# camillabelponer/dealii-slod

Hardware: AMD Instinct MI355X
Metric: SLOD patches/sec (basis built), 2D Poisson H=1/32 n_sub=8 oversampling 2 (higher is better)
Workload: dtype f64; 1 GPU; C2: 2D Poisson SLOD, H=1/32, n_sub=8, oversampling=2, D1e4 coefficient (contrast 10000), 1024 patches on rank 0 (ensemble of 1 realisations, contiguous patch blocks); patches_per_gpu=1024, parallelism=patch-sharded x1

## Files before the change

dealii-slod_amd/csrc/slod_device.h:

```cpp
#ifndef SLOD_DEVICE_H
#define SLOD_DEVICE_H

#include <hip/hip_runtime.h>
#include <stddef.h>
#include <stdint.h>

struct SlodPatchDesc
{
  int32_t  ox, oy;
  int32_t  nx, ny;
  int32_t  mx, my;
  int32_t  ccx, ccy;
  int32_t  flags;
  int32_t  m, L;
  int32_t  n_c, n_b;
  int32_t  prob;
  uint32_t plan_index;
  uint64_t out_off;
};

__host__ __device__ inline size_t slod_mt_stride(int nc_max) { return (size_t)nc_max * nc_max + 1; }

enum : int32_t
{
  SLOD_F_LOD        = 1 << 4,
  SLOD_F_TRANSPOSED = 1 << 5
};

#ifdef SLOD_ENABLE_DIAG
#define SLOD_DG(A, mask) ((A).diag & (mask))
#else
#define SLOD_DG(A, mask) 0
#endif

struct SlodPatchDiag
{
  int32_t path;
  int32_t n_cut;
  int32_t n_dropped;
  int32_t sweeps;
  double  dinf;
  double  sigma_max, sigma_min;
};

struct SlodKernelArgs
{
  const SlodPatchDesc *desc;
  const double        *coef0;
  const double        *coef1;
  size_t               coef_stride;
  int32_t              NE;
  int32_t              n_sub;
  int32_t              quirk;
  int32_t              diag;
  int32_t              debug;
  double               scale;
  double               invH2;
  double *st;
  size_t  st_stride;
  int32_t nn_max;
  double *vinv;
  size_t  v_stride;
  int32_t m_max;
  int32_t L_max;
  int32_t nv;
  double *xs;
  double *zs;
  size_t  x_stride;
  int32_t nc_max;
  double *ms;
  double *mt;
  int32_t m_tw;
  int32_t bwd_ksplit;
  int32_t nb_buf;
  int32_t nf_max;
  int32_t fuse_select;
  int32_t fuse_assemble;
  double  *basis;
  double  *premult;
  int32_t *status;
  SlodPatchDiag *pdiag;
};

enum SlodSolverKind : int32_t
{
  SLOD_K_MF   = 1,
  SLOD_K_TW   = 2,
  SLOD_K_COOP = 4,
  SLOD_K_ND   = 5
};

struct SlodTuning
{
  int solver = 0;
  int fuse_select = 1, fuse_assemble = 1, fuse_m = -1;
  int twisted = -1;
  int balance = 1;
  int bwd_ksplit = 1;
  int debug = 0;
};
struct SlodSolveChoice
{
  int    kind = 0;
  size_t lds  = 0;
  int    fuse_select = 0, fuse_assemble = 0, m_tw = 0, bwd_ksplit = 0, twisted = 0, debug = 0;
  int    v_line_pad = 0;
  size_t v_line_elems = 0;
  int    nv = 0;
  size_t v_patch_elems = 0;
};
SlodTuning slod_read_tuning();
bool       slod_choose_solver(int S, int n_sub, int m_max, int L_max, int nc_max, int nb_buf, int nf_max, size_t n_patches,
                              const SlodTuning &t, SlodSolveChoice *out);

hipError_t slod_launch_assemble(int S, const SlodKernelArgs &a, int n_patches, hipStream_t st);
hipError_t slod_launch_solve(int S, const SlodSolveChoice &c, SlodKernelArgs &a, int n_patches, hipStream_t st);
hipError_t slod_launch_solve_mf(int S, const SlodKernelArgs &a, int n_patches, size_t lds, hipStream_t st);
hipError_t slod_launch_solve_tw(int S, const SlodKernelArgs &a, int n_patches, size_t lds, hipStream_t st);
hipError_t slod_launch_solve_coop(int S, int twisted, const SlodKernelArgs &a, int n_patches, hipStream_t st);
hipError_t slod_launch_solve_nd(const SlodKernelArgs &a, int n_patches, size_t lds, hipStream_t st);
int        slod_solve_nd_cell(int S, int n_sub, int m_max, int L_max);
size_t     slod_solve_nd_scratch(int nv, int m_max, int L_max, int nc_max);
size_t     slod_solve_nd_lds_bytes(int nv, int m_max, int nc_max);
hipError_t slod_launch_select(int S, const SlodKernelArgs &a, int n_patches, int nb_max,
                              int nf_max, hipStream_t st);
size_t     slod_solve_lds_bytes(int S, int m_max, int nc_max, int twisted);
size_t     slod_solve_tw_lds_bytes(int S, int m_max, int nc_max, bool with_m = false);
size_t     slod_solve_mf_lds_bytes(int S, int m_max, int nc_max);
int        slod_lane_tile(int m_max);
int        slod_solve_mf_tiles(int S, int m_max);
size_t     slod_select_lds_bytes(int S, int nb_max, int nc_max, int nf_max);

#endif
```

dealii-slod_amd/csrc/slod_dispatch.cpp:

```cpp
#include "slod_device.h"

#include <algorithm>
#include <cstdlib>
#include <cstring>

SlodTuning slod_read_tuning()
{
  SlodTuning t;
  if (const char *sel = getenv("SLOD_SOLVE"))
    t.solver = !strcmp(sel, "mf") ? SLOD_K_MF : !strcmp(sel, "tw") ? SLOD_K_TW :
               !strcmp(sel, "coop") ? SLOD_K_COOP : !strcmp(sel, "nd") ? SLOD_K_ND : 0;
  if (const char *e = getenv("SLOD_FUSE_SELECT"))
    t.fuse_select = atoi(e) ? 1 : 0;
  if (const char *e = getenv("SLOD_FUSE_ASSEMBLE"))
    t.fuse_assemble = atoi(e) ? 1 : 0;
  if (const char *e = getenv("SLOD_FUSE_M"))
    t.fuse_m = atoi(e) ? 1 : 0;
  if (const char *e = getenv("SLOD_BWD_KSPLIT"))
    t.bwd_ksplit = atoi(e) ? 1 : 0;
  if (const char *e = getenv("SLOD_TWISTED"))
    t.twisted = atoi(e) ? 1 : 0;
  if (const char *e = getenv("SLOD_BALANCE"))
    t.balance = atoi(e) ? 1 : 0;
  if (const char *e = getenv("SLOD_DEBUG"))
    t.debug = atoi(e) ? 1 : 0;
  return t;
}

int slod_lane_tile(int m_max)
{
  static const int tiles[] = {2, 3, 4, 5, 6, 8, 10, 12, 14};
  for (int t : tiles)
    if (8 * t >= m_max)
      return t;
  return 0;
}

bool slod_choose_solver(int S, int n_sub, int m_max, int L_max, int nc_max, int nb_buf, int nf_max, size_t n_patches,
                        const SlodTuning &t_in, SlodSolveChoice *out)
{
  const size_t    lds_max = 160 * 1024;
  SlodSolveChoice c;
  const int       nd_nv = slod_solve_nd_cell(S, n_sub, m_max, L_max);
  SlodTuning      t     = t_in;
  if (t.solver == SLOD_K_ND && nd_nv == 0)
    t.solver = 0;
  c.debug = t.debug;
  const int  wt = slod_lane_tile(m_max);
  const bool lane_tile_fits = wt > 0 && wt >= 2 * S - 1;
  const auto want = [&](int k) { return t.solver == 0 || t.solver == k; };
  const size_t lds_sel = slod_select_lds_bytes(S, nb_buf, nc_max, nf_max);
  const bool   mf_fits = slod_solve_mf_tiles(S, m_max) > 0 && slod_solve_mf_lds_bytes(S, m_max, nc_max) <= lds_max;
  const bool   tw_fits = lane_tile_fits && slod_solve_tw_lds_bytes(S, m_max, nc_max) <= lds_max;
  if (nd_nv > 0 && t.solver == SLOD_K_ND)
    {
      c.kind          = SLOD_K_ND;
      c.nv            = nd_nv;
      c.lds           = slod_solve_nd_lds_bytes(nd_nv, m_max, nc_max);
      c.v_patch_elems = slod_solve_nd_scratch(nd_nv, m_max, L_max, nc_max);
      c.fuse_assemble = t.fuse_assemble ? 1 : 0;
      c.fuse_select   = 0;
    }
  else if (mf_fits && (t.solver == SLOD_K_MF || (t.solver == 0 && !tw_fits && !lane_tile_fits)))
    {
      c.kind          = SLOD_K_MF;
      c.lds           = slod_solve_mf_lds_bytes(S, m_max, nc_max);
      c.v_line_pad    = 16 * slod_solve_mf_tiles(S, m_max);
      c.v_line_elems  = (size_t)c.v_line_pad * c.v_line_pad;
      c.fuse_assemble = (S == 1 && t.fuse_assemble) ? 1 : 0;
      c.fuse_select   = (S == 1 && t.fuse_select && lds_sel <= lds_max) ? 1 : 0;
      if (c.fuse_select && lds_sel > c.lds)
        c.lds = lds_sel;
    }
  else if (want(SLOD_K_TW) && tw_fits)
    {
      c.kind          = SLOD_K_TW;
      c.lds           = slod_solve_tw_lds_bytes(S, m_max, nc_max);
      c.v_line_pad    = 8 * wt;
      c.v_line_elems  = (size_t)64 * wt * wt;
      c.fuse_assemble = (S == 1 && t.fuse_assemble) ? 1 : 0;
      c.fuse_select = (S == 1 && t.fuse_select && lds_sel <= 64 * 1024) ? 1 : 0;
      if (S == 1 && t.fuse_m != 0 && nc_max <= 32 && 8 * wt <= 48)
        {
          const size_t sel    = c.fuse_select ? lds_sel : 0;
          const size_t with_m = std::max(slod_solve_tw_lds_bytes(S, m_max, nc_max, true), sel);
          if (std::min<size_t>(4, lds_max / with_m) == std::min<size_t>(4, lds_max / std::max(c.lds, sel)))
            {
              c.m_tw = 1;
              c.lds  = slod_solve_tw_lds_bytes(S, m_max, nc_max, true);
            }
        }
      if (c.fuse_select && lds_sel > c.lds)
        c.lds = lds_sel;
      c.bwd_ksplit = (t.bwd_ksplit && 8 * wt <= 48 && nc_max <= 32) ? 1 : 0;
    }
  else if (t.solver == 0 || t.solver == SLOD_K_COOP || !lane_tile_fits)
    {
      int tw = t.twisted >= 0 ? t.twisted : (n_patches < 3 * 256 ? 1 : 0);
      if (slod_solve_lds_bytes(S, m_max, nc_max, tw) > lds_max)
        tw = 0;
      if (slod_solve_lds_bytes(S, m_max, nc_max, tw) > lds_max || (m_max + 15) / 16 > 7)
        return false;
      c.kind       = SLOD_K_COOP;
      c.twisted    = tw;
      c.lds        = slod_solve_lds_bytes(S, m_max, nc_max, tw);
      c.v_line_pad = m_max;
      c.v_line_elems = (size_t)m_max * m_max;
    }
  else
    return false;
  if (!c.fuse_select && lds_sel > lds_max)
    return false;
  *out = c;
  return true;
}

hipError_t slod_launch_solve(int S, const SlodSolveChoice &c, SlodKernelArgs &a, int n_patches, hipStream_t st)
{
  a.m_tw          = c.m_tw;
  a.bwd_ksplit    = c.bwd_ksplit;
  a.fuse_select   = c.fuse_select;
  a.fuse_assemble = c.fuse_assemble;
  a.debug         = c.debug;
  switch (c.kind)
    {
      case SLOD_K_MF:
        return slod_launch_solve_mf(S, a, n_patches, c.lds, st);
      case SLOD_K_TW:
        return slod_launch_solve_tw(S, a, n_patches, c.lds, st);
      case SLOD_K_COOP:
        return slod_launch_solve_coop(S, c.twisted, a, n_patches, st);
      case SLOD_K_ND:
        a.nv = c.nv;
        return slod_launch_solve_nd(a, n_patches, c.lds, st);
      default:
        return hipErrorInvalidValue;
    }
}
```

dealii-slod_amd/csrc/slod_select.hip.h:

```cpp
#ifndef SLOD_SELECT_HIP_H
#define SLOD_SELECT_HIP_H
#include <type_traits>
#include "slod_common.hip.h"

namespace
{

  template <int S, bool OWN = false>
  __device__ __forceinline__ void select_patch(const SlodKernelArgs &A, const int nb_max, const int nf_max,
                                               const int patch, double *smem, const double *mpre = nullptr)
  {
    const SlodPatchDesc d   = A.desc[patch];
    const int           tid = threadIdx.x;
    const int           nc = d.n_c, nb = d.n_b, n = A.n_sub;
    const int           ncm = A.nc_max, ldm = ncm + 1;
    const int           mm = A.m_max, ncs = A.nc_max;
    const bool          tr  = (d.flags & SLOD_F_TRANSPOSED) != 0;
    const bool          lod = (d.flags & SLOD_F_LOD) != 0;
    const int           npx = d.nx + 1, nn = npx * (d.ny + 1), nf = S * nn;

    double *Ms   = smem;
    double *Vj   = Ms + ncm * ldm;
    double *BD   = Vj + ncm * ncm;
    double *phis = BD;
    double *sig  = BD + max(nb_max * ncm, nf_max);
    double *utg  = sig + ncm;
    double *gam  = utg + ncm;
    double *cvec = gam + ncm;
    double *rowk = cvec + ncm;
    double *red  = rowk + ncm;
    const int vst = max(nb_max, 160);
    double *vcol = red + 8;
    int    *colk = reinterpret_cast<int *>(vcol + 2 * vst);
    int    *ord  = colk + 2 * ncm;
    int    *flag = ord + ncm;
    int    *pcol = flag + 4;

    const double *st    = A.st + (size_t)patch * A.st_stride;
    const double *xg    = A.xs + (size_t)patch * A.x_stride;
    const size_t  xline = (size_t)mm * ncs;
    const int     wave = tid >> 6, lane = tid & 63, grp = tid >> 4, l16 = tid & 15;

    auto xrow = [&](int ix, int iy, int comp) -> const double * {
      if (ix <= 0 || ix >= d.nx || iy <= 0 || iy >= d.ny)
        return nullptr;
      const int l = tr ? ix - 1 : iy - 1, pos = tr ? iy - 1 : ix - 1;
      return xg + (size_t)l * xline + (size_t)(pos * S + comp) * ncs;
    };
    auto ptw = [&](int ix, int iy, int comp, int col) -> double {
      if (S == 1)
        {
          const int jx = ix - colk[col] * n, jy = iy - colk[ncm + col] * n;
          if (jx < 0 || jx > n || jy < 0 || jy > n)
            return 0.0;
          return ((jx == 0 || jx == n) ? 1.0 : 2.0) * ((jy == 0 || jy == n) ? 1.0 : 2.0);
        }
      return pt_weight<S>(d, n, A.quirk, ix, iy, comp, col);
    };
    auto block_sum = [&](double v) -> double {
      for (int off = 32; off > 0; off >>= 1)
        v += __shfl_xor(v, off, 64);
      __syncthreads();
      if (lane == 0)
        red[wave] = v;
      __syncthreads();
      return red[0] + red[1] + red[2] + red[3];
    };

    for (int c = tid; c < nc; c += 256)
      {
        int kx, ky;
        cell_of_col(d, c / S, kx, ky);
        colk[c]       = kx;
        colk[ncm + c] = ky;
      }
    __syncthreads();

    const bool stamping = (SLOD_DG(A, (1 << 20))) && tid == 0 && A.nc_max * A.nc_max >= 12;
    double    *msd      = A.ms + (size_t)patch * A.nc_max * A.nc_max;
    double     tph[3]   = {0.0, 0.0, 0.0};
    double     tlast    = stamping ? (double)wall_clock64() : 0.0;
    auto       stamp    = [&](int i) {
      if (stamping)
        msd[i] = tlast = (double)wall_clock64();
    };
    auto tacc = [&](int i) {
      if (stamping)
        {
          const double now = (double)wall_clock64();
          tph[i] += now - tlast;
          tlast = now;
        }
    };

    const bool m_given = mpre != nullptr;
    if (m_given)
      for (int idx = tid; idx < nc * nc; idx += 256)
        Ms[(idx / nc) * ldm + (idx % nc)] = mpre[idx];
    for (int idx = tid; idx < ((SLOD_DG(A, 64)) || m_given ? 0 : nc * (nc + 1) / 2); idx += 256)
      {
        int a = (int)((2.0f * nc + 1.0f - sqrtf((2.0f * nc + 1.0f) * (2.0f * nc + 1.0f) - 8.0f * idx)) * 0.5f);
        a     = min(max(a, 0), nc - 1);
        while (a > 0 && a * (2 * nc - a + 1) / 2 > idx)
          --a;
        while (a + 1 < nc && (a + 1) * (2 * nc - a) / 2 <= idx)
          ++a;
        const int b  = a + idx - a * (2 * nc - a + 1) / 2;
        const int kx = colk[a], ky = colk[ncm + a];
        double    acc = 0.0;
        if (S == 1 || !A.quirk)
          {
            const int ca = a % S;
            for (int jy0 = 0; jy0 <= n; jy0 += 3)
              for (int jx0 = 0; jx0 <= n; jx0 += 9)
                {
                  double xv[3][9];
#pragma unroll
                  for (int ry = 0; ry < 3; ++ry)
                    {
                      const int iy  = ky * n + jy0 + ry;
                      const int iyc = min(max(iy, 1), d.ny - 1);
#pragma unroll
                      for (int rx = 0; rx < 9; ++rx)
                        {
                          const int ix  = kx * n + jx0 + rx;
                          const int ixc = min(max(ix, 1), d.nx - 1);
                          const int l = tr ? ixc - 1 : iyc - 1, pos = tr ? iyc - 1 : ixc - 1;
                          xv[ry][rx]  = xg[(size_t)l * xline + (size_t)(pos * S + ca) * ncs + b];
                        }
                    }
#pragma unroll
                  for (int ry = 0; ry < 3; ++ry)
                    {
                      const int    jy = jy0 + ry, iy = ky * n + jy;
                      const double wy = (jy <= n && iy > 0 && iy < d.ny) ? ((jy == 0 || jy == n) ? 1.0 : 2.0) : 0.0;
                      double       part = 0.0;
#pragma unroll
                      for (int rx = 0; rx < 9; ++rx)
                        {
                          const int    jx = jx0 + rx, ix = kx * n + jx;
                          const double w = (jx <= n && ix > 0 && ix < d.nx) ? ((jx == 0 || jx == n) ? 1.0 : 2.0) : 0.0;
                          part           = fma(w, xv[ry][rx], part);
                        }
                      acc = fma(wy, part, acc);
                    }
                }
          }
        else
          {
            for (int jy = 0; jy <= n; ++jy)
              for (int jx = 0; jx <= n; ++jx)
                {
                  const int ix = kx * n + jx, iy = ky * n + jy;
#pragma unroll
                  for (int c = 0; c < S; ++c)
                    {
                      const double *xr = xrow(ix, iy, c);
                      if (xr)
                        acc = fma(pt_weight<S>(d, n, A.quirk, ix, iy, c, a), xr[b], acc);
                    }
                }
          }
        Ms[a * ldm + b] = acc * A.scale * A.invH2;
        Ms[b * ldm + a] = acc * A.scale * A.invH2;
      }
    __syncthreads();
    stamp(3);

    if (nc * nc <= 1024)
      {
        double mv[4];
        int    mi[4], mj[4];
#pragma unroll
        for (int e = 0; e < 4; ++e)
          {
            const int idx = tid + 256 * e;
            mi[e]         = idx / nc;
            mj[e]         = idx - mi[e] * nc;
            mv[e]         = (idx < nc * nc) ? Ms[mi[e] * ldm + mj[e]] : 0.0;
            if (idx < nc * nc && mi[e] == 0)
              cvec[mj[e]] = mv[e];
          }
        __syncthreads();
        for (int k = 0; k < ((SLOD_DG(A, 128)) ? 0 : nc); ++k)
          {
            const double *rk  = (k & 1) ? rowk : cvec;
            double       *rn  = (k & 1) ? cvec : rowk;
            const double  piv = rk[k];
            if (tid == 0 && !(piv > 0.0) && !SLOD_DG(A, -1))
              atomicOr(A.status, 2);
            const double p = fast_rcp(piv);
#pragma unroll
            for (int e = 0; e < 4; ++e)
              if (tid + 256 * e < nc * nc)
                {
                  const int    i = mi[e], j = mj[e];
                  const double ri = rk[i], rj = rk[j];
                  double       v;
                  if (i == k)
                    v = (j == k) ? -p : rj * p;
                  else if (j == k)
                    v = ri * p;
                  else
                    v = fma(-(ri * rj), p, mv[e]);
                  mv[e] = v;
                  if (i == k + 1)
                    rn[j] = v;
                }
            __syncthreads();
          }
#pragma unroll
        for (int e = 0; e < 4; ++e)
          if (tid + 256 * e < nc * nc)
            Ms[mi[e] * ldm + mj[e]] = -mv[e];
        __syncthreads();
      }
    else
      {
        for (int k = 0; k < ((SLOD_DG(A, 128)) ? 0 : nc); ++k)
          {
            for (int j = tid; j < nc; j += 256)
              rowk[j] = Ms[k * ldm + j];
            __syncthreads();
            const double piv = rowk[k];
            if (tid == 0 && !(piv > 0.0) && !SLOD_DG(A, -1))
              atomicOr(A.status, 2);
            const double p = fast_rcp(piv);
            for (int idx = tid; idx < nc * nc; idx += 256)
              {
                const int    i = idx / nc, j = idx - i * nc;
                const double ri = rowk[i], rj = rowk[j];
                double       v;
                if (i == k)
                  v = (j == k) ? -p : rj * p;
                else if (j == k)
                  v = ri * p;
                else
                  v = fma(-(ri * rj), p, Ms[i * ldm + j]);
                Ms[i * ldm + j] = v;
              }
            __syncthreads();
          }
        for (int idx = tid; idx < nc * nc; idx += 256)
          {
            const int i = idx / nc, j = idx - i * nc;
            Ms[i * ldm + j] = -Ms[i * ldm + j];
          }
        __syncthreads();
      }
    stamp(4);
    double *Ds = Ms;

    for (int dsel = 0; dsel < S; ++dsel)
      {
        for (int j = tid; j < nc; j += 256)
          gam[j] = (j == dsel) ? 1.0 : 0.0;
        SlodPatchDiag pdg = {0, 0, 0, 0, 0.0, 0.0, 0.0};
        if (!lod)
          {
            pdg.path = 1;
            const int nn1 = nc - 1;
            auto      cix = [&](int j) { return j < dsel ? j : j + 1; };
            const int nbuf = nb_max;
            int       nr   = 0;
            bool      need_svd = true, singular = false, did_qr = false;
            int       filled = 0;
            auto qr_sweep = [&](auto &a, const int rows, const bool last) __attribute__((always_inline)) {
              constexpr int RQ = sizeof(a[0]) / sizeof(double);
            if (grp == 0)
              {
                double nx0 = 0.0;
#pragma unroll
                for (int i = 0; i < RQ; ++i)
                  {
                    nx0 = fma(a[0][i], a[0][i], nx0);
                    if (l16 + 16 * i < rows)
                      vcol[l16 + 16 * i] = a[0][i];
                  }
                nx0 = group16_sum(nx0);
                if (l16 == 0)
                  sig[0] = nx0;
              }
            __syncthreads();
            for (int k = 0; k < nn1; ++k)
              {
                const double *vc    = vcol + (k & 1) * vst;
                double       *vn    = vcol + ((k + 1) & 1) * vst;
                const double  sigma = sig[k & 1];
                const bool    act   = sigma > 0.0;
                if (!act && last)
                  singular = true;
                const double x0    = vc[k];
                const double sq    = act ? sigma * fast_rsqrt(sigma) : 0.0;
                const double alpha = (x0 >= 0.0) ? -sq : sq;
                const double v0    = x0 - alpha;
                const double beta  = act ? fast_rcp(sigma - alpha * x0) : 0.0;
                double       vr[RQ];
#pragma unroll
                for (int i = 0; i < RQ; ++i)
                  {
                    const int r = l16 + 16 * i;
                    vr[i]       = (r == k) ? v0 : ((r > k && r < rows) ? vc[r] : 0.0);
                  }
#pragma unroll
                for (int sl = 0; sl < 2; ++sl)
                  {
                    const int j = grp + 16 * sl;
                    if (j == k)
                      {
#pragma unroll
                        for (int i = 0; i < RQ; ++i)
                          {
                            const int r = l16 + 16 * i;
                            a[sl][i]    = (r == k) ? (act ? alpha : a[sl][i]) : (r > k ? 0.0 : a[sl][i]);
                          }
                      }
                    else if (j > k && j <= nn1)
                      {
                        double sd = 0.0;
#pragma unroll
                        for (int i = 0; i < RQ; ++i)
                          sd = fma(vr[i], a[sl][i], sd);
                        sd = group16_sum(sd) * beta;
#pragma unroll
                        for (int i = 0; i < RQ; ++i)
                          a[sl][i] = fma(-sd, vr[i], a[sl][i]);
                        if (j == k + 1 && j < nn1)
                          {
                            double nxt = 0.0;
#pragma unroll
                            for (int i = 0; i < RQ; ++i)
                              {
                                const int r = l16 + 16 * i;
                                if (r > k)
                                  nxt = fma(a[sl][i], a[sl][i], nxt);
                                if (r < rows)
                                  vn[r] = a[sl][i];
                              }
                            nxt = group16_sum(nxt);
                            if (l16 == 0)
                              sig[(k + 1) & 1] = nxt;
                          }
                      }
                  }
                __syncthreads();
              }
            };
            const bool onepass = nb <= 160 && nb > 96 && nc <= 32 && (nbuf & 15) == 0 && !(SLOD_DG(A, (512 | 262144)));
            double     aq[2][10];
            for (int r0 = 0; r0 < nb;)
              {
                const int take = min(nb - r0, nbuf - filled);
                {
                  constexpr int U = 2;
                  for (int idx0 = tid; idx0 < ((SLOD_DG(A, 256)) ? 0 : take * nc); idx0 += 256 * U)
                    {
                      double sv[U][3][S], xv[U][3][S], acc[U];
                      int    dst[U];
#pragma unroll
                      for (int u = 0; u < U; ++u)
                        {
                          const int  idx = idx0 + 256 * u;
                          const bool ok  = idx < take * nc;
                          const int  br = ok ? idx / nc : 0, c = ok ? idx - br * nc : 0;
                          const int  bi = r0 + br;
                          const int  bn = bi / S, ca = bi - bn * S;
                          int        ix, iy;
                          boundary_node(d, bn, ix, iy);
                          acc[u] = -A.scale * ptw(ix, iy, ca, c);
                          dst[u] = ok ? (filled + br) * ncm + c : -1;
                          const bool hor = (iy == 0 || iy == d.ny);
                          const int  ndx = ix == 0 ? 1 : -1, ndy = iy == 0 ? 1 : -1;
#pragma unroll
                          for (int e = -1; e <= 1; ++e)
                            {
                              const int  dx = hor ? e : ndx, dy = hor ? ndy : e;
                              const int  jx = ix + dx, jy = iy + dy;
                              const bool in = (jx > 0 && jx < d.nx && jy > 0 && jy < d.ny);
                              const int  jxc = min(max(jx, 1), d.nx - 1), jyc = min(max(jy, 1), d.ny - 1);
                              const int  dir = (dy + 1) * 3 + dx + 1;
                              const int  l = tr ? jxc - 1 : jyc - 1, pos = tr ? jyc - 1 : jxc - 1;
#pragma unroll
                              for (int cb = 0; cb < S; ++cb)
                                {
                                  const double svv = st[(size_t)((dir * S + ca) * S + cb) * A.nn_max + ix + iy * npx];
                                  sv[u][e + 1][cb] = in ? svv : 0.0;
                                  xv[u][e + 1][cb] = xg[(size_t)l * xline + (size_t)(pos * S + cb) * ncs + c];
                                }
                            }
                        }
#pragma unroll
                      for (int u = 0; u < U; ++u)
                        {
#pragma unroll
                          for (int e = 0; e < 3; ++e)
#pragma unroll
                            for (int cb = 0; cb < S; ++cb)
                              acc[u] = fma(sv[u][e][cb], xv[u][e][cb], acc[u]);
                          if (dst[u] >= 0)
                            BD[dst[u]] = acc[u];
                        }
                    }
                }
                __syncthreads();
                tacc(0);
                for (int ti = wave; 16 * ti < take; ti += 4)
                  {
                    const int  arow = filled + 16 * ti + (lane & 15);
                    const bool aok  = 16 * ti + (lane & 15) < take;
                    double4_t  acc[4];
#pragma unroll
                    for (int tj = 0; tj < 4; ++tj)
                      acc[tj] = double4_t{0.0, 0.0, 0.0, 0.0};
                    for (int k = 0; k < nc; k += 4)
                      {
                        const int    kk = k + (lane >> 4);
                        const double av = (aok && kk < nc) ? BD[arow * ncm + kk] : 0.0;
#pragma unroll
                        for (int tj = 0; tj < 4; ++tj)
                          if (16 * tj < nc)
                            {
                              const int    col = 16 * tj + (lane & 15);
                              const double bv  = (kk < nc && col < nc) ? Ds[kk * ldm + col] : 0.0;
                              acc[tj]          = __builtin_amdgcn_mfma_f64_16x16x4f64(av, bv, acc[tj], 0, 0, 0);
                            }
                      }
#pragma unroll
                    for (int tj = 0; tj < 4; ++tj)
#pragma unroll
                      for (int r = 0; r < 4; ++r)
                        {
                          const int rr = 16 * ti + (lane >> 4) + 4 * r, col = 16 * tj + (lane & 15);
                          if (rr < take && col < nc)
                            BD[(filled + rr) * ncm + col] = acc[tj][r];
                        }
                  }
                __syncthreads();
                tacc(1);
                if (onepass)
                  {
#pragma unroll
                    for (int sl = 0; sl < 2; ++sl)
                      {
                        const int j = grp + 16 * sl, cj = j < nn1 ? cix(j) : dsel;
#pragma unroll
                        for (int i = 0; i < 10; ++i)
                          {
                            const int r = l16 + 16 * i;
                            if (r >= r0 && r < r0 + take)
                              aq[sl][i] = (j <= nn1) ? BD[(r - r0) * ncm + cj] : 0.0;
                            else if (r0 == 0)
                              aq[sl][i] = 0.0;
                          }
                      }
                    r0 += take;
                    __syncthreads();
                    continue;
                  }
                r0 += take;
                const int rows = filled + take;
                nr             = rows;
                if (rows < nn1 || (SLOD_DG(A, 512)))
                  {
                    filled = rows;
                    if (filled >= nbuf)
                      break;
                    continue;
                  }
                did_qr = true;
                if (rows <= 96 && nc <= 32)
                  {
                    double a[2][6];
#pragma unroll
                    for (int sl = 0; sl < 2; ++sl)
                      {
                        const int j = grp + 16 * sl;
                        const int cj = j < nn1 ? cix(j) : dsel;
#pragma unroll
                        for (int i = 0; i < 6; ++i)
                          {
                            const int r = l16 + 16 * i;
                            a[sl][i]    = (j <= nn1 && r < rows) ? BD[r * ncm + cj] : 0.0;
                          }
                      }
                    qr_sweep(a, rows, r0 >= nb);
#pragma unroll
                    for (int sl = 0; sl < 2; ++sl)
                      {
                        const int j = grp + 16 * sl;
                        const int cj = j < nn1 ? cix(j) : dsel;
#pragma unroll
                        for (int i = 0; i < 6; ++i)
                          {
                            const int r = l16 + 16 * i;
                            if (j <= nn1 && r < rows)
                              BD[r * ncm + cj] = a[sl][i];
                          }
                      }
                  }
                else
                  {
                    {
                      double part = 0.0;
                      for (int r = tid; r < rows; r += 256)
                        {
                          const double x = BD[r * ncm + cix(0)];
                          part           = fma(x, x, part);
                        }
                      const double s00 = block_sum(part);
                      if (tid == 0)
                        sig[0] = s00;
                      __syncthreads();
                    }
                    for (int k = 0; k < nn1; ++k)
                      {
                        const int    ck    = cix(k);
                        const double sigma = sig[k & 1];
                        if (!(sigma > 0.0))
                          {
                            if (r0 >= nb)
                              singular = true;
                            if (k + 1 < nn1)
                              {
                                double part = 0.0;
                                for (int r = k + 1 + tid; r < rows; r += 256)
                                  {
                                    const double x = BD[r * ncm + cix(k + 1)];
                                    part           = fma(x, x, part);
                                  }
                                const double sn = block_sum(part);
                                if (tid == 0)
                                  sig[(k + 1) & 1] = sn;
                              }
                            __syncthreads();
                            continue;
                          }
                        const double x0    = BD[k * ncm + ck];
                        const double sq    = sigma * fast_rsqrt(sigma);
                        const double alpha = (x0 >= 0.0) ? -sq : sq;
                        const double v0    = x0 - alpha;
                        const double beta  = fast_rcp(sigma - alpha * x0);
                        if constexpr (OWN)
                          {
                            constexpr int NRL = 10;
                            double        vr[NRL];
    #pragma unroll
                            for (int i = 0; i < NRL; ++i)
                              {
                                const int    r = k + l16 + 16 * i;
                                const double x = BD[min(r, rows - 1) * ncm + ck];
                                vr[i]          = (r < rows) ? ((r == k) ? v0 : x) : 0.0;
                              }
                            for (int t = grp; t < nn1 - k; t += 16)
                              {
                                const int cj = (t == nn1 - k - 1) ? dsel : cix(k + 1 + t);
                                double    xj[NRL];
    #pragma unroll
                                for (int i = 0; i < NRL; ++i)
                                  xj[i] = BD[min(k + l16 + 16 * i, rows - 1) * ncm + cj];
                                double sd = 0.0;
    #pragma unroll
                                for (int i = 0; i < NRL; ++i)
                                  sd = (k + l16 + 16 * i < rows) ? fma(vr[i], xj[i], sd) : sd;
                                sd = group16_sum(sd) * beta;
                                double nxt = 0.0;
    #pragma unroll
                                for (int i = 0; i < NRL; ++i)
                                  {
                                    const int r = k + l16 + 16 * i;
                                    if (r < rows)
                                      {
                                        const double nv  = fma(-sd, vr[i], xj[i]);
                                        BD[r * ncm + cj] = nv;
                                        if (r > k)
                                          nxt = fma(nv, nv, nxt);
                                      }
                                  }
                                if (t == 0 && k + 1 < nn1)
                                  {
                                    nxt = group16_sum(nxt);
                                    if (l16 == 0)
                                      sig[(k + 1) & 1] = nxt;
                                  }
                              }
                          }
                        else
                          {
                            for (int t = grp; t < nn1 - k; t += 16)
                              {
                                const int cj = (t == nn1 - k - 1) ? dsel : cix(k + 1 + t);
                                double    sd = 0.0;
                                for (int r = k + l16; r < rows; r += 16)
                                  {
                                    const double vr = (r == k) ? v0 : BD[r * ncm + ck];
                                    sd              = fma(vr, BD[r * ncm + cj], sd);
                                  }
                                sd = group16_sum(sd) * beta;
                                double nxt = 0.0;
                                for (int r = k + l16; r < rows; r += 16)
                                  {
                                    const double vr = (r == k) ? v0 : BD[r * ncm + ck];
                                    const double nv = fma(-sd, vr, BD[r * ncm + cj]);
                                    BD[r * ncm + cj] = nv;
                                    if (r > k)
                                      nxt = fma(nv, nv, nxt);
                                  }
                                if (t == 0 && k + 1 < nn1)
                                  {
                                    nxt = group16_sum(nxt);
                                    if (l16 == 0)
                                      sig[(k + 1) & 1] = nxt;
                                  }
                              }
                          }
                        __syncthreads();
                        if (tid == 0)
                          BD[k * ncm + ck] = alpha;
                      }
                    for (int idx = tid; idx < nn1 * nn1; idx += 256)
                      {
                        const int r = idx / nn1, j = idx - r * nn1;
                        if (r > j)
                          BD[r * ncm + cix(j)] = 0.0;
                      }
                    for (int r = nn1 + tid; r < rows; r += 256)
                      for (int j = 0; j < nn1; ++j)
                        BD[r * ncm + cix(j)] = 0.0;
                  }
                __syncthreads();
                tacc(2);
                filled = nn1;
                nr     = nn1;
              }
            if (onepass)
              {
                did_qr = true;
                qr_sweep(aq, nb, true);
#pragma unroll
                for (int sl = 0; sl < 2; ++sl)
                  {
                    const int j = grp + 16 * sl, cj = j < nn1 ? cix(j) : dsel;
#pragma unroll
                    for (int i = 0; i < 2; ++i)
                      {
                        const int r = l16 + 16 * i;
                        if (j <= nn1 && r < nn1)
                          BD[r * ncm + cj] = aq[sl][i];
                      }
                  }
                __syncthreads();
                tacc(2);
                nr = nn1;
              }
            if (did_qr && !(SLOD_DG(A, 512)))
              {
                if (!singular)
                  {
                    double    fr = 0.0, fi = 0.0;
                    const int l8 = tid & 7;
                    for (int j = tid >> 3; j < nn1; j += 32)
                      {
                        const int cj = cix(j);
                        if (l8 == 0)
                          Vj[j * nn1 + j] = 1.0 / BD[j * ncm + cj];
                        for (int i = j - 1; i >= 0; --i)
                          {
                            const double rd = fast_rcp(BD[i * ncm + cix(i)]);
                            double       sa = 0.0;
                            for (int k2 = i + 1 + l8; k2 <= j; k2 += 8)
                              sa = fma(BD[i * ncm + cix(k2)], Vj[k2 * nn1 + j], sa);
                            sa += dpp_rot<0xB1>(sa);
                            sa += dpp_rot<0x4E>(sa);
                            sa += dpp_rot<0x141>(sa);
                            if (l8 == 0)
                              Vj[i * nn1 + j] = -sa * rd;
                          }
                        for (int i = l8; i <= j; i += 8)
                          {
                            const double r = BD[i * ncm + cj], x = Vj[i * nn1 + j];
                            fr             = fma(r, r, fr);
                            fi             = fma(x, x, fi);
                          }
                      }
                    const double nr2 = block_sum(fr), ni2 = block_sum(fi);
                    double       del = 0.0;
                    if (tid < nn1)
                      {
                        for (int j = tid; j < nn1; ++j)
                          del = fma(-Vj[tid * nn1 + j], BD[j * ncm + dsel], del);
                        rowk[tid] = del;
                      }
                    double dmax = fabs(del);
                    for (int off = 32; off > 0; off >>= 1)
                      dmax = fmax(dmax, __shfl_xor(dmax, off, 64));
                    __syncthreads();
                    if (lane == 0)
                      red[4 + wave] = dmax;
                    __syncthreads();
                    const double dinf = fmax(fmax(red[4], red[5]), fmax(red[6], red[7]));
                    pdg.dinf          = dinf;
                    if (nr2 * ni2 < 1e14 && dinf < 0.5 - 1e-9)
                      {
                        need_svd = false;
                        if (tid < nn1)
                          gam[cix(tid)] = rowk[tid];
                      }
                  }
              }
            if (stamping)
              {
                msd[5] = tph[0];
                msd[6] = tph[1];
                msd[7] = tph[2];
              }
            stamp(8);
            if (need_svd && !(SLOD_DG(A, (512 | 4096))))
              {
                pdg.path = 2;
                const bool tposed = did_qr && nbuf >= 2 * nn1 + 1;
                double    *Wm     = BD;
                int        wr     = nr;
                int        pb     = 0;
                for (int j = tid; j < nn1; j += 256)
                  pcol[j] = j;
                if (tposed && nc <= 32 && !(SLOD_DG(A, 65536)))
                  {
                    double a[2][2];
                    bool   fin[2] = {false, false};
#pragma unroll
                    for (int sl = 0; sl < 2; ++sl)
                      {
                        const int j = grp + 16 * sl, cj = j < nn1 ? cix(j) : dsel;
#pragma unroll
                        for (int i = 0; i < 2; ++i)
                          {
                            const int r = l16 + 16 * i;
                            a[sl][i]    = (j <= nn1 && r < nn1) ? BD[r * ncm + cj] : 0.0;
                          }
                        const double nrm = group16_sum(fma(a[sl][0], a[sl][0], a[sl][1] * a[sl][1]));
                        if (j < nn1 && l16 == 0)
                          sig[j] = nrm;
                      }
                    __syncthreads();
                    for (int k = 0; k < nn1; ++k)
                      {
                        const int    *pc  = pcol + pb * ncm;
                        int          *pn  = pcol + (1 - pb) * ncm;
                        const double *cnc = (k & 1) ? utg : sig;
                        double       *cnn = (k & 1) ? sig : utg;
                        int    p;
                        double best;
                        {
                          const bool pin = lane >= k && lane < nn1;
                          double     v   = cnc[pc[pin ? lane : k]];
                          int        q   = pin ? lane : 64;
                          v              = pin ? v : -1.0;
                          auto step = [&](auto CTRL_) __attribute__((always_inline)) {
                            constexpr int CTRL = decltype(CTRL_)::value;
                            const double  ov   = dpp_rot<CTRL>(v);
                            const int     oq   = __builtin_amdgcn_mov_dpp(q, CTRL, 0xf, 0xf, false);
                            const bool    take = (ov > v) | ((ov == v) & (oq < q));
                            v                  = take ? ov : v;
                            q                  = take ? oq : q;
                          };
                          step(std::integral_constant<int, 0x128>{});
                          step(std::integral_constant<int, 0x124>{});
                          step(std::integral_constant<int, 0x122>{});
                          step(std::integral_constant<int, 0x121>{});
                          const int    q0 = __builtin_amdgcn_readlane(q, 0), q1 = __builtin_amdgcn_readlane(q, 16);
                          const double v0 = __hiloint2double(__builtin_amdgcn_readlane(__double2hiint(v), 0),
                                                             __builtin_amdgcn_readlane(__double2loint(v), 0));
                          const double v1 = __hiloint2double(__builtin_amdgcn_readlane(__double2hiint(v), 16),
                                                             __builtin_amdgcn_readlane(__double2loint(v), 16));
                          const bool   hi = v1 > v0;
                          best            = hi ? v1 : v0;
                          p               = hi ? q1 : q0;
                        }
                        if (!(best > 0.0))
                          break;
                        const int cp = pc[p];
                        if (tid < nn1)
                          pn[tid] = (tid == k) ? cp : (tid == p ? pc[k] : pc[tid]);
                        const int    ccp   = cix(cp);
                        const double x0    = BD[k * ncm + ccp];
                        const double sq    = best * fast_rsqrt(best);
                        const double alpha = (x0 >= 0.0) ? -sq : sq;
                        const double v0    = x0 - alpha;
                        const double beta  = fast_rcp(best - alpha * x0);
                        double       vr[2];
#pragma unroll
                        for (int i = 0; i < 2; ++i)
                          {
                            const int r = l16 + 16 * i;
                            vr[i]       = (r == k) ? v0 : ((r > k && r < nn1) ? BD[r * ncm + ccp] : 0.0);
                          }
#pragma unroll
                        for (int sl = 0; sl < 2; ++sl)
                          {
                            const int j = grp + 16 * sl, cj = j < nn1 ? cix(j) : dsel;
                            if (j > nn1 || fin[sl])
                              continue;
                            if (j == cp)
                              {
#pragma unroll
                                for (int i = 0; i < 2; ++i)
                                  {
                                    const int r = l16 + 16 * i;
                                    a[sl][i]    = (r == k) ? alpha : (r > k ? 0.0 : a[sl][i]);
                                  }
                                fin[sl] = true;
                              }
                            else
                              {
                                const double sd = group16_sum(fma(vr[0], a[sl][0], vr[1] * a[sl][1])) * beta;
                                double       nrm = 0.0;
#pragma unroll
                                for (int i = 0; i < 2; ++i)
                                  {
                                    const int r = l16 + 16 * i;
                                    a[sl][i]    = fma(-sd, vr[i], a[sl][i]);
                                    if (r > k)
                                      nrm = fma(a[sl][i], a[sl][i], nrm);
                                    if (r >= k && r < nn1)
                                      BD[r * ncm + cj] = a[sl][i];
                                  }
                                nrm = group16_sum(nrm);
                                if (j < nn1 && l16 == 0)
                                  cnn[j] = nrm;
                              }
                          }
                        __syncthreads();
                        pb ^= 1;
                      }
#pragma unroll
                    for (int sl = 0; sl < 2; ++sl)
                      {
                        const int j = grp + 16 * sl, cj = j < nn1 ? cix(j) : dsel;
#pragma unroll
                        for (int i = 0; i < 2; ++i)
                          {
                            const int r = l16 + 16 * i;
                            if (j <= nn1 && r < nn1)
                              BD[r * ncm + cj] = a[sl][i];
                          }
                      }
                  }
                __syncthreads();
                if (stamping && A.nc_max * A.nc_max >= 16)
                  msd[14] = (double)wall_clock64();
                const int *pc = pcol + pb * ncm;
                if (tposed)
                  {
                    Wm = BD + (size_t)nn1 * ncm;
                    for (int idx = tid; idx < nn1 * nn1; idx += 256)
                      {
                        const int i = idx / nn1, j = idx - i * nn1;
                        Wm[i * ncm + j] = (j <= i) ? BD[j * ncm + cix(pc[i])] : 0.0;
                      }
                    for (int j = tid; j < nn1; j += 256)
                      Wm[nn1 * ncm + j] = BD[j * ncm + dsel];
                    wr = nn1;
                  }
                const int wru = tposed ? wr + 1 : wr;
                auto wcol = [&](int j) { return tposed ? j : cix(j); };
                const int nev = (nn1 + 1) & ~1;
                for (int idx = tid; idx < nn1 * nn1; idx += 256)
                  Vj[idx] = ((idx / nn1) == (idx % nn1)) ? 1.0 : 0.0;
                double fro = 0.0;
                for (int idx = tid; idx < wr * nn1; idx += 256)
                  {
                    const double w = Wm[(idx / nn1) * ncm + wcol(idx % nn1)];
                    fro            = fma(w, w, fro);
                  }
                const double tiny = 1e-22 * block_sum(fro);
                if (nev / 2 <= 16 && (SLOD_DG(A, 131072)))
                  {
                    if (wave == 0)
                      {
                        const int l4 = lane & 3, pr = lane >> 2;
                        for (int sweep = 0; sweep < ((SLOD_DG(A, 8192)) ? 3 : 40); ++sweep)
                          {
                            bool any = false;
                            for (int round = 0; round < nev - 1; ++round)
                              {
                                int pa, pb2;
                                if (pr == 0)
                                  {
                                    pa  = nev - 1;
                                    pb2 = round;
                                  }
                                else
                                  {
                                    pa  = round + pr;
                                    pa  = pa >= nev - 1 ? pa - (nev - 1) : pa;
                                    pb2 = round - pr;
                                    pb2 = pb2 < 0 ? pb2 + (nev - 1) : pb2;
                                  }
                                const bool valid = pr < nev / 2 && pa < nn1 && pb2 < nn1;
                                const int  p = valid ? (pa < pb2 ? pa : pb2) : 0, q = valid ? (pa < pb2 ? pb2 : pa) : 0;
                                const int  cp = wcol(p), cq = wcol(q);
                                double     app = 0, aqq = 0, apq = 0;
                                for (int r = l4; r < wr; r += 4)
                                  {
                                    const double wp = Wm[r * ncm + cp], wq = Wm[r * ncm + cq];
                                    app = fma(wp, wp, app);
                                    aqq = fma(wq, wq, aqq);
                                    apq = fma(wp, wq, apq);
                                  }
                                app += dpp_rot<0xB1>(app);
                                aqq += dpp_rot<0xB1>(aqq);
                                apq += dpp_rot<0xB1>(apq);
                                app += dpp_rot<0x4E>(app);
                                aqq += dpp_rot<0x4E>(aqq);
                                apq += dpp_rot<0x4E>(apq);
                                const bool rot = valid && !(apq == 0.0 || apq * apq <= 1e-30 * (app * aqq) ||
                                                            fmax(app, aqq) <= tiny);
                                if (rot)
                                  {
                                    const double dd = aqq - app;
                                    const double hh = fma(dd, dd, 4.0 * apq * apq);
                                    const double hy = hh * fast_rsqrt(hh);
                                    const double t  = (dd >= 0.0 ? 2.0 : -2.0) * apq * fast_rcp(fabs(dd) + hy);
                                    const double cs = fast_rsqrt(fma(t, t, 1.0)), sn = cs * t;
                                    for (int r = l4; r < wru; r += 4)
                                      {
                                        const double wp = Wm[r * ncm + cp], wq = Wm[r * ncm + cq];
                                        Wm[r * ncm + cp] = cs * wp - sn * wq;
                                        Wm[r * ncm + cq] = sn * wp + cs * wq;
                                      }
                                    for (int r = l4; r < (tposed ? 0 : nn1); r += 4)
                                      {
                                        const double vp = Vj[r * nn1 + p], vq = Vj[r * nn1 + q];
                                        Vj[r * nn1 + p] = cs * vp - sn * vq;
                                        Vj[r * nn1 + q] = sn * vp + cs * vq;
                                      }
                                    any = true;
                                  }
                              }
                            if (!__any(any))
                              break;
                          }
                      }
                    __syncthreads();
                  }
                else
                  for (int sweep = 0; sweep < ((SLOD_DG(A, 8192)) ? 3 : 40); ++sweep)
                    {
                      if (tid == 0)
                        flag[0] = 0;
                      __syncthreads();
                      for (int round = 0; round < nev - 1; ++round)
                        {
                          for (int pr = grp; pr < nev / 2; pr += 16)
                            {
                              int pa, pb;
                              if (pr == 0)
                                {
                                  pa = nev - 1;
                                  pb = round;
                                }
                              else
                                {
                                  pa = round + pr;
                                  pa = pa >= nev - 1 ? pa - (nev - 1) : pa;
                                  pb = round - pr;
                                  pb = pb < 0 ? pb + (nev - 1) : pb;
                                }
                              if (pa >= nn1 || pb >= nn1)
                                continue;
                              const int p = pa < pb ? pa : pb, q = pa < pb ? pb : pa;
                              const int cp = wcol(p), cq = wcol(q);
                              double    app = 0, aqq = 0, apq = 0;
                              for (int r = l16; r < wr; r += 16)
                                {
                                  const double wp = Wm[r * ncm + cp], wq = Wm[r * ncm + cq];
                                  app = fma(wp, wp, app);
                                  aqq = fma(wq, wq, aqq);
                                  apq = fma(wp, wq, apq);
                                }
                              app = group16_sum(app);
                              aqq = group16_sum(aqq);
                              apq = group16_sum(apq);
                              if (apq == 0.0 || apq * apq <= 1e-30 * (app * aqq) || fmax(app, aqq) <= tiny)
                                continue;
                              const double dd = aqq - app;
                              const double hh = fma(dd, dd, 4.0 * apq * apq);
                              const double hy = hh * fast_rsqrt(hh);
                              const double t  = (dd >= 0.0 ? 2.0 : -2.0) * apq * fast_rcp(fabs(dd) + hy);
                              const double cs = fast_rsqrt(fma(t, t, 1.0)), sn = cs * t;
                              for (int r = l16; r < wru; r += 16)
                                {
                                  const double wp = Wm[r * ncm + cp], wq = Wm[r * ncm + cq];
                                  Wm[r * ncm + cp] = cs * wp - sn * wq;
                                  Wm[r * ncm + cq] = sn * wp + cs * wq;
                                }
                              for (int r = l16; r < (tposed ? 0 : nn1); r += 16)
                                {
                                  const double vp = Vj[r * nn1 + p], vq = Vj[r * nn1 + q];
                                  Vj[r * nn1 + p] = cs * vp - sn * vq;
                                  Vj[r * nn1 + q] = sn * vp + cs * vq;
                                }
                              if (l16 == 0)
                                flag[0] = 1;
                            }
                          __syncthreads();
                        }
                      const int any = flag[0];
                      __syncthreads();
                      ++pdg.sweeps;
                      if (!any)
                        break;
                    }
                if (stamping && A.nc_max * A.nc_max >= 16)
                  msd[15] = (double)wall_clock64();
                for (int j = tid; j < nn1; j += 256)
                  {
                    const int cj = wcol(j);
                    double    ss = 0, wb = 0;
                    for (int r = 0; r < wr; ++r)
                      {
                        const double w = Wm[r * ncm + cj];
                        ss             = fma(w, w, ss);
                        if (!tposed)
                          wb = fma(w, BD[r * ncm + dsel], wb);
                      }
                    if (tposed)
                      wb = Wm[nn1 * ncm + j];
                    sig[j] = ss;
                    utg[j] = wb;
                  }
                __syncthreads();
                auto tvec = [&](int a2, int j) { return tposed ? Wm[a2 * ncm + j] : Vj[a2 * nn1 + j]; };
                for (int j = tid; j < nn1; j += 256)
                  {
                    const double sj = sig[j];
                    int          rank = 0;
                    for (int i = 0; i < nn1; ++i)
                      {
                        const double si = sig[i];
                        rank += (si > sj || (si == sj && i < j)) ? 1 : 0;
                      }
                    ord[rank] = j;
                  }
                __syncthreads();
                {
                  const double s0 = sig[ord[0]];
                  pdg.sigma_max   = s0;
                  pdg.sigma_min   = sig[ord[nn1 - 1]];
                  if (wave == 0)
                    pdg.n_cut = __popcll(__ballot(tid < nn1 && !(sig[min(tid, nn1 - 1)] > 1e-15 * s0)));
                  for (int j = tid; j < nn1; j += 256)
                    utg[j] = (sig[j] > 1e-15 * s0) ? utg[j] / sig[j] : 0.0;
                }
                __syncthreads();
                double del = 0.0;
                if (tid < nn1)
                  for (int j = 0; j < nn1; ++j)
                    del = fma(-tvec(tid, j), utg[j], del);
                if (nn1 <= 64)
                  {
                    if (wave == 0)
                      {
                        for (int r = nn1 - 1; r >= 0; --r)
                          {
                            double dmax = (tid < nn1) ? fabs(del) : 0.0;
                            for (int off = 32; off > 0; off >>= 1)
                              dmax = fmax(dmax, __shfl_xor(dmax, off, 64));
                            pdg.dinf = dmax;
                            if (dmax < 0.5)
                              break;
                            const int j = ord[r];
                            if (tid < nn1)
                              del = fma(tvec(tid, j), utg[j], del);
                            ++pdg.n_dropped;
                          }
                        if (pdg.n_dropped == nn1)
                          {
                            double dmax = (tid < nn1) ? fabs(del) : 0.0;
                            for (int off = 32; off > 0; off >>= 1)
                              dmax = fmax(dmax, __shfl_xor(dmax, off, 64));
                            pdg.dinf = dmax;
                          }
                      }
                  }
                else
                  for (int r = nn1 - 1; r >= 0; --r)
                    {
                      double dmax = (tid < nn1) ? fabs(del) : 0.0;
                      for (int off = 32; off > 0; off >>= 1)
                        dmax = fmax(dmax, __shfl_xor(dmax, off, 64));
                      __syncthreads();
                      if (lane == 0)
                        red[4 + wave] = dmax;
                      __syncthreads();
                      const double dinf = fmax(fmax(red[4], red[5]), fmax(red[6], red[7]));
                      pdg.dinf = dinf;
                      if (dinf < 0.5)
                        break;
                      const int j = ord[r];
                      if (tid < nn1)
                        del = fma(tvec(tid, j), utg[j], del);
                      ++pdg.n_dropped;
                    }
                if (tid < nn1)
                  gam[cix(pc[tid])] = del;
              }
          }
        if (tid == 0 && A.pdiag)
          A.pdiag[(size_t)d.plan_index * S + dsel] = pdg;
        __syncthreads();
        stamp(9);
        for (int i = tid; i < nc; i += 256)
          {
            double acc = 0.0;
            for (int j = 0; j < nc; ++j)
              acc = fma(Ds[i * ldm + j], gam[j], acc);
            cvec[i] = acc;
          }
        __syncthreads();
        double ssq = 0.0;
        for (int dof = tid; dof < ((SLOD_DG(A, 1024)) ? 0 : nf); dof += 256)
          {
            const int     node = dof / S, comp = dof - node * S;
            const int     ix = node % npx, iy = node / npx;
            const double *xr  = xrow(ix, iy, comp);
            double        acc = 0.0;
            if (xr)
              for (int j0 = 0; j0 < nc; j0 += 13)
                {
                  double xv[13];
#pragma unroll
                  for (int e = 0; e < 13; ++e)
                    xv[e] = xr[min(j0 + e, nc - 1)];
#pragma unroll
                  for (int e = 0; e < 13; ++e)
                    acc = fma(xv[e], (j0 + e < nc) ? cvec[j0 + e] : 0.0, acc);
                }
            phis[dof] = acc;
            ssq       = fma(acc, acc, ssq);
          }
        const double nrm = sqrt(block_sum(ssq));
        double      *ob  = A.basis + d.out_off + (size_t)dsel * nf;
        double      *op  = A.premult + d.out_off + (size_t)dsel * nf;
        for (int dof = tid; dof < nf; dof += 256)
          {
            const double v = phis[dof] / nrm;
            phis[dof]      = v;
            ob[dof]        = v;
          }
        __syncthreads();
        stamp(10);
        for (int dof = tid; dof < ((SLOD_DG(A, 2048)) ? 0 : nf); dof += 256)
          {
            const int  node = dof / S, comp = dof - node * S;
            const int  ix = node % npx, iy = node / npx;
            const bool dom = (ix == 0 && (d.flags & 1)) || (ix == d.nx && (d.flags & 2)) ||
                             (iy == 0 && (d.flags & 4)) || (iy == d.ny && (d.flags & 8));
            double sv[9][S];
#pragma unroll
            for (int dir = 0; dir < 9; ++dir)
#pragma unroll
              for (int cb = 0; cb < S; ++cb)
                sv[dir][cb] = st[(size_t)((dir * S + comp) * S + cb) * A.nn_max + node];
            double acc = 0.0;
#pragma unroll
            for (int dy = -1; dy <= 1; ++dy)
#pragma unroll
              for (int dx = -1; dx <= 1; ++dx)
                {
                  const int  jx = ix + dx, jy = iy + dy;
                  const bool in = !(jx < 0 || jx > d.nx || jy < 0 || jy > d.ny);
                  const int  jn = min(max(jx, 0), d.nx) + min(max(jy, 0), d.ny) * npx;
                  const int  dir = (dy + 1) * 3 + dx + 1;
#pragma unroll
                  for (int cb = 0; cb < S; ++cb)
                    acc = fma(in ? sv[dir][cb] : 0.0, phis[jn * S + cb], acc);
                }
            if (dom)
              acc = phis[dof];
            op[dof] = acc;
          }
        __syncthreads();
        stamp(11);
      }
  }
}

#endif
```

Baseline: 1.095 million patches/s.

## Keep SVD pivot columns in registers and use a 16-lane-group Jacobi sweep path

Adds an svd_regs tuning flag, on by default for S==1 transposed patches with nc<=32. When it is set, pivoted QR keeps the column permutation in a per-lane register updated with readlane instead of double-buffering it through LDS. The one-sided Jacobi sweep is replaced by a path where each 16-lane group handles one rotation pair, holding two rows in registers and reducing with group16_sum, and convergence is checked through per-wave flags once per sweep. It also skips initialising Vj in the transposed case. The aim is to cut LDS traffic and barriers in the SVD/select stage, at the cost of a __syncthreads per round and possible numerical differences because fp contraction is turned off in that path.

```diff
diff --git a/dealii-slod_amd/csrc/slod_device.h b/dealii-slod_amd/csrc/slod_device.h
--- a/dealii-slod_amd/csrc/slod_device.h
+++ b/dealii-slod_amd/csrc/slod_device.h
@@ -72,6 +72,7 @@
   double *mt;
   int32_t m_tw;
   int32_t bwd_ksplit;
+  int32_t svd_regs;
   int32_t nb_buf;
   int32_t nf_max;
   int32_t fuse_select;
@@ -97,13 +98,14 @@
   int twisted = -1;
   int balance = 1;
   int bwd_ksplit = 1;
+  int svd_regs = 1;
   int debug = 0;
 };
 struct SlodSolveChoice
 {
   int    kind = 0;
   size_t lds  = 0;
-  int    fuse_select = 0, fuse_assemble = 0, m_tw = 0, bwd_ksplit = 0, twisted = 0, debug = 0;
+  int    fuse_select = 0, fuse_assemble = 0, m_tw = 0, bwd_ksplit = 0, svd_regs = 0, twisted = 0, debug = 0;
   int    v_line_pad = 0;
   size_t v_line_elems = 0;
   int    nv = 0;
diff --git a/dealii-slod_amd/csrc/slod_dispatch.cpp b/dealii-slod_amd/csrc/slod_dispatch.cpp
--- a/dealii-slod_amd/csrc/slod_dispatch.cpp
+++ b/dealii-slod_amd/csrc/slod_dispatch.cpp
@@ -18,6 +18,8 @@
     t.fuse_m = atoi(e) ? 1 : 0;
   if (const char *e = getenv("SLOD_BWD_KSPLIT"))
     t.bwd_ksplit = atoi(e) ? 1 : 0;
+  if (const char *e = getenv("SLOD_SVD_REGS"))
+    t.svd_regs = atoi(e) ? 1 : 0;
   if (const char *e = getenv("SLOD_TWISTED"))
     t.twisted = atoi(e) ? 1 : 0;
   if (const char *e = getenv("SLOD_BALANCE"))
@@ -46,6 +48,7 @@
   if (t.solver == SLOD_K_ND && nd_nv == 0)
     t.solver = 0;
   c.debug = t.debug;
+  c.svd_regs = t.svd_regs ? 1 : 0;
   const int  wt = slod_lane_tile(m_max);
   const bool lane_tile_fits = wt > 0 && wt >= 2 * S - 1;
   const auto want = [&](int k) { return t.solver == 0 || t.solver == k; };
@@ -119,6 +122,7 @@
 {
   a.m_tw          = c.m_tw;
   a.bwd_ksplit    = c.bwd_ksplit;
+  a.svd_regs      = c.svd_regs;
   a.fuse_select   = c.fuse_select;
   a.fuse_assemble = c.fuse_assemble;
   a.debug         = c.debug;
diff --git a/dealii-slod_amd/csrc/slod_select.hip.h b/dealii-slod_amd/csrc/slod_select.hip.h
--- a/dealii-slod_amd/csrc/slod_select.hip.h
+++ b/dealii-slod_amd/csrc/slod_select.hip.h
@@ -723,6 +723,7 @@
                 int        pb     = 0;
                 for (int j = tid; j < nn1; j += 256)
                   pcol[j] = j;
+                const bool regs = S == 1 && tposed && nc <= 32 && A.svd_regs;
                 if (tposed && nc <= 32 && !(SLOD_DG(A, 65536)))
                   {
                     double a[2][2];
@@ -742,6 +743,7 @@
                           sig[j] = nrm;
                       }
                     __syncthreads();
+                    int mypc = lane < nn1 ? lane : 0;
                     for (int k = 0; k < nn1; ++k)
                       {
                         const int    *pc  = pcol + pb * ncm;
@@ -752,7 +754,7 @@
                         double best;
                         {
                           const bool pin = lane >= k && lane < nn1;
-                          double     v   = cnc[pc[pin ? lane : k]];
+                          double     v   = regs ? cnc[mypc] : cnc[pc[pin ? lane : k]];
                           int        q   = pin ? lane : 64;
                           v              = pin ? v : -1.0;
                           auto step = [&](auto CTRL_) __attribute__((always_inline)) {
@@ -778,21 +780,41 @@
                         }
                         if (!(best > 0.0))
                           break;
-                        const int cp = pc[p];
-                        if (tid < nn1)
-                          pn[tid] = (tid == k) ? cp : (tid == p ? pc[k] : pc[tid]);
-                        const int    ccp   = cix(cp);
-                        const double x0    = BD[k * ncm + ccp];
+                        int    cp;
+                        double x0, vr[2];
+                        if (regs)
+                          {
+                            cp           = __builtin_amdgcn_readlane(mypc, p);
+                            const int ck = __builtin_amdgcn_readlane(mypc, k);
+                            mypc         = (lane == k) ? cp : (lane == p ? ck : mypc);
+                            const int ccp = cix(cp);
+                            x0            = BD[k * ncm + ccp];
+                            vr[0]         = BD[min(l16, nn1 - 1) * ncm + ccp];
+                            vr[1]         = BD[min(l16 + 16, nn1 - 1) * ncm + ccp];
+                          }
+                        else
+                          {
+                            cp = pc[p];
+                            if (tid < nn1)
+                              pn[tid] = (tid == k) ? cp : (tid == p ? pc[k] : pc[tid]);
+                            const int ccp = cix(cp);
+                            x0            = BD[k * ncm + ccp];
+#pragma unroll
+                            for (int i = 0; i < 2; ++i)
+                              {
+                                const int r = l16 + 16 * i;
+                                vr[i]       = (r > k && r < nn1) ? BD[r * ncm + ccp] : 0.0;
+                              }
+                          }
                         const double sq    = best * fast_rsqrt(best);
                         const double alpha = (x0 >= 0.0) ? -sq : sq;
                         const double v0    = x0 - alpha;
                         const double beta  = fast_rcp(best - alpha * x0);
-                        double       vr[2];
 #pragma unroll
                         for (int i = 0; i < 2; ++i)
                           {
                             const int r = l16 + 16 * i;
-                            vr[i]       = (r == k) ? v0 : ((r > k && r < nn1) ? BD[r * ncm + ccp] : 0.0);
+                            vr[i]       = (r == k) ? v0 : ((r > k && r < nn1) ? vr[i] : 0.0);
                           }
 #pragma unroll
                         for (int sl = 0; sl < 2; ++sl)
@@ -830,8 +852,11 @@
                               }
                           }
                         __syncthreads();
-                        pb ^= 1;
-                      }
+                        if (!regs)
+                          pb ^= 1;
+                      }
+                    if (regs && tid < nn1)
+                      pcol[tid] = mypc;
 #pragma unroll
                     for (int sl = 0; sl < 2; ++sl)
                       {
@@ -864,7 +889,7 @@
                 const int wru = tposed ? wr + 1 : wr;
                 auto wcol = [&](int j) { return tposed ? j : cix(j); };
                 const int nev = (nn1 + 1) & ~1;
-                for (int idx = tid; idx < nn1 * nn1; idx += 256)
+                for (int idx = tid; idx < (tposed ? 0 : nn1 * nn1); idx += 256)
                   Vj[idx] = ((idx / nn1) == (idx % nn1)) ? 1.0 : 0.0;
                 double fro = 0.0;
                 for (int idx = tid; idx < wr * nn1; idx += 256)
@@ -873,75 +898,76 @@
                     fro            = fma(w, w, fro);
                   }
                 const double tiny = 1e-22 * block_sum(fro);
-                if (nev / 2 <= 16 && (SLOD_DG(A, 131072)))
-                  {
-                    if (wave == 0)
-                      {
-                        const int l4 = lane & 3, pr = lane >> 2;
-                        for (int sweep = 0; sweep < ((SLOD_DG(A, 8192)) ? 3 : 40); ++sweep)
-                          {
-                            bool any = false;
-                            for (int round = 0; round < nev - 1; ++round)
+                if (regs)
+                  {
+                    const int  o0 = min(l16, nn1) * ncm, o1 = min(l16 + 16, nn1) * ncm;
+                    const bool u0 = l16 < wru, u1 = l16 + 16 < wru;
+                    const bool d0 = l16 < wr, d1 = l16 + 16 < wr;
+                    for (int sweep = 0; sweep < ((SLOD_DG(A, 8192)) ? 3 : 40); ++sweep)
+                      {
+                        bool anyt = false;
+                        for (int round = 0; round < nev - 1; ++round)
+                          {
+#pragma clang fp contract(off)
+                            int pa, pb;
+                            if (grp == 0)
                               {
-                                int pa, pb2;
-                                if (pr == 0)
-                                  {
-                                    pa  = nev - 1;
-                                    pb2 = round;
-                                  }
-                                else
-                                  {
-                                    pa  = round + pr;
-                                    pa  = pa >= nev - 1 ? pa - (nev - 1) : pa;
-                                    pb2 = round - pr;
-                                    pb2 = pb2 < 0 ? pb2 + (nev - 1) : pb2;
-                                  }
-                                const bool valid = pr < nev / 2 && pa < nn1 && pb2 < nn1;
-                                const int  p = valid ? (pa < pb2 ? pa : pb2) : 0, q = valid ? (pa < pb2 ? pb2 : pa) : 0;
-                                const int  cp = wcol(p), cq = wcol(q);
-                                double     app = 0, aqq = 0, apq = 0;
-                                for (int r = l4; r < wr; r += 4)
-                                  {
-                                    const double wp = Wm[r * ncm + cp], wq = Wm[r * ncm + cq];
-                                    app = fma(wp, wp, app);
-                                    aqq = fma(wq, wq, aqq);
-                                    apq = fma(wp, wq, apq);
-                                  }
-                                app += dpp_rot<0xB1>(app);
-                                aqq += dpp_rot<0xB1>(aqq);
-                                apq += dpp_rot<0xB1>(apq);
-                                app += dpp_rot<0x4E>(app);
-                                aqq += dpp_rot<0x4E>(aqq);
-                                apq += dpp_rot<0x4E>(apq);
-                                const bool rot = valid && !(apq == 0.0 || apq * apq <= 1e-30 * (app * aqq) ||
-                                                            fmax(app, aqq) <= tiny);
-                                if (rot)
-                                  {
-                                    const double dd = aqq - app;
-                                    const double hh = fma(dd, dd, 4.0 * apq * apq);
-                                    const double hy = hh * fast_rsqrt(hh);
-                                    const double t  = (dd >= 0.0 ? 2.0 : -2.0) * apq * fast_rcp(fabs(dd) + hy);
-                                    const double cs = fast_rsqrt(fma(t, t, 1.0)), sn = cs * t;
-                                    for (int r = l4; r < wru; r += 4)
-                                      {
-                                        const double wp = Wm[r * ncm + cp], wq = Wm[r * ncm + cq];
-                                        Wm[r * ncm + cp] = cs * wp - sn * wq;
-                                        Wm[r * ncm + cq] = sn * wp + cs * wq;
-                                      }
-                                    for (int r = l4; r < (tposed ? 0 : nn1); r += 4)
-                                      {
-                                        const double vp = Vj[r * nn1 + p], vq = Vj[r * nn1 + q];
-                                        Vj[r * nn1 + p] = cs * vp - sn * vq;
-                                        Vj[r * nn1 + q] = sn * vp + cs * vq;
-                                      }
-                                    any = true;
-                                  }
+                                pa = nev - 1;
+                                pb = round;
                               }
-                            if (!__any(any))
-                              break;
-                          }
-                      }
-                    __syncthreads();
+                            else
+                              {
+                                pa = round + grp;
+                                pa = pa >= nev - 1 ? pa - (nev - 1) : pa;
+                                pb = round - grp;
+                                pb = pb < 0 ? pb + (nev - 1) : pb;
+                              }
+                            const bool valid = (grp < nev / 2) & (pa < nn1) & (pb < nn1);
+                            const int  p = valid ? (pa < pb ? pa : pb) : 0, q = valid ? (pa < pb ? pb : pa) : 0;
+                            double     wp0 = Wm[o0 + p], wq0 = Wm[o0 + q], wp1 = Wm[o1 + p], wq1 = Wm[o1 + q];
+                            wp0 = (valid & u0) ? wp0 : 0.0;
+                            wq0 = (valid & u0) ? wq0 : 0.0;
+                            wp1 = (valid & u1) ? wp1 : 0.0;
+                            wq1 = (valid & u1) ? wq1 : 0.0;
+                            const double xp0 = d0 ? wp0 : 0.0, xq0 = d0 ? wq0 : 0.0;
+                            const double xp1 = d1 ? wp1 : 0.0, xq1 = d1 ? wq1 : 0.0;
+                            const double app = group16_sum(fma(xp1, xp1, fma(xp0, xp0, 0.0)));
+                            const double aqq = group16_sum(fma(xq1, xq1, fma(xq0, xq0, 0.0)));
+                            const double apq = group16_sum(fma(xp1, xq1, fma(xp0, xq0, 0.0)));
+                            const bool   rot = valid & !((apq == 0.0) | (apq * apq <= 1e-30 * (app * aqq)) |
+                                                       (fmax(app, aqq) <= tiny));
+                            const double dd = aqq - app;
+                            const double hh = fma(dd, dd, (4.0 * apq) * apq);
+                            const double t  = ((dd >= 0.0 ? 2.0 : -2.0) * apq) * fast_rcp(fma(hh, fast_rsqrt(hh), fabs(dd)));
+                            const double cs = fast_rsqrt(fma(t, t, 1.0)), sn = cs * t;
+                            const double np0 = fma(cs, wp0, -(sn * wq0)), nq0 = fma(sn, wp0, cs * wq0);
+                            const double np1 = fma(cs, wp1, -(sn * wq1)), nq1 = fma(sn, wp1, cs * wq1);
+                            if (rot & u0)
+                              {
+                                Wm[o0 + p] = np0;
+                                Wm[o0 + q] = nq0;
+                              }
+                            if (rot & u1)
+                              {
+                                Wm[o1 + p] = np1;
+                                Wm[o1 + q] = nq1;
+                              }
+                            anyt |= rot;
+                            if (round == nev - 2)
+                              {
+                                const int wany = __any(anyt) ? 1 : 0;
+                                if (lane == 0)
+                                  flag[wave] = wany;
+                              }
+                            __syncthreads();
+                          }
+                        const int any = flag[0] | flag[1] | flag[2] | flag[3];
+                        if (nev == 2)
+                          __syncthreads();
+                        ++pdg.sweeps;
+                        if (!any)
+                          break;
+                      }
                   }
                 else
                   for (int sweep = 0; sweep < ((SLOD_DG(A, 8192)) ? 3 : 40); ++sweep)
```

New measurement: 1.112 million patches/s (median of 6 runs). 1.6% higher.
